# visinf/da-sac

Hardware: AMD Instinct MI355X
Metric: train images/sec (769x769, 19-cls, RN101 DeepLabv2, K=3) (higher is better)
Workload: dtype f32

## Files before the change

### da-sac_amd/csrc/conv_igemm.hip

```cpp
#include "common.hpp"

#include <atomic>
#include <cstdlib>
#include <type_traits>

namespace dasac {

typedef float f32x16 __attribute__((ext_vector_type(16)));
typedef float f32x4 __attribute__((ext_vector_type(4)));

constexpr int kBK = 16;
constexpr int kThreads = 256;
constexpr int kInvalid = 1 << 20;
constexpr int kSkWorkersPerCu = 3;
constexpr int kSkWorkers = kNumCu * kSkWorkersPerCu;
constexpr int kTileSlots = kNumCu * 4;
constexpr int kTailSlots = 2048;

#ifdef DASAC_TRACE_TILES
__device__ unsigned long long* g_tile_trace = nullptr;
__device__ __forceinline__ void trace_stamp(int slot) {
  if (g_tile_trace && threadIdx.x == 0) g_tile_trace[(size_t)blockIdx.x * 8 + slot] = __builtin_amdgcn_s_memtime();
}
#define DASAC_STAMP(slot) trace_stamp(slot)
#else
#define DASAC_STAMP(slot)
#endif

struct GemmGeom {
  int H, W, CxHW;
  int OH, OW, stride;
  int Npix;
  int n_tile0;
  int M, Mpad, Kpad;
  int OutH, OutW, ostride;
  unsigned x_bytes, w_bytes, z_bytes, out_bytes;
};

struct Epilogue {
  const float* shift;
  const float* res;
  const float* mask;
  int relu;
  const unsigned* mbits;
  unsigned* obits;
  int w32;
  float* stats;
};

constexpr unsigned kPoison = 0xFFFFFFFFu;
constexpr int64_t kMaxTensorBytes = (1ll << 32) - 4096;
constexpr int kRsrcFlags = 0x00020000;
typedef unsigned int u32x4 __attribute__((ext_vector_type(4)));

__device__ __forceinline__ __amdgpu_buffer_rsrc_t make_rsrc(const void* p, unsigned bytes) {
  return __builtin_amdgcn_make_buffer_rsrc(const_cast<void*>(p), 0, (int)bytes, kRsrcFlags);
}
__device__ __forceinline__ float buf_f32(__amdgpu_buffer_rsrc_t r, unsigned voff, int soff) {
  return __uint_as_float(__builtin_amdgcn_raw_buffer_load_b32(r, voff, soff, 0));
}

constexpr int kAuxSc1 = 16;
__device__ __forceinline__ f32x4 buf_f32x4_sc1(__amdgpu_buffer_rsrc_t r, unsigned voff, int soff) {
  const u32x4 v = __builtin_amdgcn_raw_buffer_load_b128(r, voff, soff, kAuxSc1);
  return f32x4{__uint_as_float(v.x), __uint_as_float(v.y), __uint_as_float(v.z), __uint_as_float(v.w)};
}
__device__ __forceinline__ f32x4 buf_f32x4(__amdgpu_buffer_rsrc_t r, unsigned voff, int soff) {
  const u32x4 v = __builtin_amdgcn_raw_buffer_load_b128(r, voff, soff, 0);
  return f32x4{__uint_as_float(v.x), __uint_as_float(v.y), __uint_as_float(v.z), __uint_as_float(v.w)};
}

#if __has_builtin(__builtin_amdgcn_writelane)
template <int LANE>
__device__ __forceinline__ int writelane_c(int val, int old) {
  return __builtin_amdgcn_writelane(val, LANE, old);
}
#else
extern "C" __device__ int dasac_llvm_writelane(int val, int lane, int old) __asm("llvm.amdgcn.writelane.i32");
template <int LANE>
__device__ __forceinline__ int writelane_c(int val, int old) {
  return dasac_llvm_writelane(val, LANE, old);
}
#endif
__device__ __forceinline__ int put_mask_rows(int rg, unsigned long long ballot, int acc) {
  const int lo = (int)(unsigned)ballot, hi = (int)(unsigned)(ballot >> 32);
  switch (rg) {
#define DASAC_ROW_(RG)                                               \
  case RG:                                                           \
    acc = writelane_c<(RG & 3) + 8 * (RG >> 2)>(lo, acc);            \
    acc = writelane_c<(RG & 3) + 8 * (RG >> 2) + 4>(hi, acc);        \
    break;
    DASAC_ROW_(0) DASAC_ROW_(1) DASAC_ROW_(2) DASAC_ROW_(3) DASAC_ROW_(4) DASAC_ROW_(5) DASAC_ROW_(6) DASAC_ROW_(7)
    DASAC_ROW_(8) DASAC_ROW_(9) DASAC_ROW_(10) DASAC_ROW_(11) DASAC_ROW_(12) DASAC_ROW_(13) DASAC_ROW_(14) DASAC_ROW_(15)
#undef DASAC_ROW_
  }
  return acc;
}

typedef __bf16 bf16x8 __attribute__((ext_vector_type(8)));
typedef __bf16 bf16x2 __attribute__((ext_vector_type(2)));
typedef float f32x2 __attribute__((ext_vector_type(2)));
__device__ __forceinline__ bf16x8 as_bf16x8(f32x4 v) { return __builtin_bit_cast(bf16x8, v); }
__device__ __forceinline__ unsigned pack_bf16(float a, float b) {
  return __builtin_bit_cast(unsigned, __builtin_convertvector((f32x2){a, b}, bf16x2));
}
__device__ __forceinline__ void split_bf16(f32x4 v0, f32x4 v1, f32x4& heads, f32x4& tails) {
  const float v[8] = {v0.x, v0.y, v0.z, v0.w, v1.x, v1.y, v1.z, v1.w};
#pragma unroll
  for (int p = 0; p < 4; ++p) {
    const unsigned h = pack_bf16(v[2 * p], v[2 * p + 1]);
    const float t0 = v[2 * p] - __uint_as_float(h << 16), t1 = v[2 * p + 1] - __uint_as_float(h & 0xffff0000u);
    heads[p] = __uint_as_float(h);
    tails[p] = __uint_as_float(pack_bf16(t0, t1));
  }
}

template <int CTRL>
__device__ __forceinline__ float dpp_add(float v) {
  return v + __int_as_float(__builtin_amdgcn_update_dpp(0, __float_as_int(v), CTRL, 0xf, 0xf, true));
}
__device__ __forceinline__ float half_wave_sum(float v) {
  v = dpp_add<0xB1>(v);
  v = dpp_add<0x4E>(v);
  v = dpp_add<0x141>(v);
  v = dpp_add<0x140>(v);
  return v + __shfl_xor(v, 16, 64);
}

template <int BM, int BN, int WAVES_M, int BK, bool FAST, int SK, bool X3, int BITS = 0>
__global__ __launch_bounds__(kThreads, SK == 1 ? kSkWorkersPerCu : 4) void conv_gemm(const float* __restrict__ X, const float* __restrict__ Wp,
                                                      const int4* __restrict__ tab, float* __restrict__ Out,
                                                      GemmGeom g, Epilogue ep, int m_tiles, int n_tiles,
                                                      float* __restrict__ partial, int* __restrict__ flags, int tail_tiles,
                                                      int tail_split) {
  constexpr bool STREAMK = SK == 1;
  constexpr bool TAIL = SK == 2;
  constexpr bool HANDOFF = STREAMK || TAIL;
  constexpr int WAVES_N = 4 / WAVES_M;
  constexpr int WM = BM / WAVES_M, WN = BN / WAVES_N;
  constexpr int TM = WM / 32, TN = WN / 32;
  constexpr int KQ = BK / 4;
  constexpr int A_VEC = KQ * BM;
  constexpr int A_PER_T = (A_VEC + kThreads - 1) / kThreads;
  constexpr int B_Q_PASS = kThreads / BN > 0 ? kThreads / BN : 1;
  constexpr int B_QUADS = KQ / B_Q_PASS;
  constexpr int ACC_REGS = TM * TN * 16;
  static_assert(TM >= 1 && TN >= 1 && BN <= kThreads && KQ % B_Q_PASS == 0, "tile shape");
  static_assert(!X3 || (BK == 16 && BN == 128), "split-bf16 path: one 16-deep MFMA block per K-step, a k octet per thread");

  __shared__ f32x4 sA[2][KQ * BM];
  __shared__ f32x4 sB[2][KQ * BN];
  __shared__ __attribute__((aligned(16))) float s_shift[BM];
  __shared__ unsigned s_vo[BN];
  __shared__ __attribute__((aligned(16))) unsigned s_mbits[BITS == 2 ? (BN / 32) * BM : 4];

  const int t = threadIdx.x, lane = t & 63;
  const int wave = __builtin_amdgcn_readfirstlane(t >> 6);
  const int wm = wave / WAVES_N, wn = wave % WAVES_N;
  const int li = lane & 31, lh = lane >> 5;

  const __amdgpu_buffer_rsrc_t rx = make_rsrc(X, g.x_bytes);
  const __amdgpu_buffer_rsrc_t rw = make_rsrc(Wp, g.w_bytes);

  const int OHW = g.OH * g.OW;
  const int planeHW = g.H * g.W;
  const int bcol = t % BN;
  const int bq0 = __builtin_amdgcn_readfirstlane(t / BN);
  const int a_step_bytes = KQ * g.Mpad * 16;
  const int KT = g.Kpad / BK;
  const int OutHW = g.OutH * g.OutW;
  const __amdgpu_buffer_rsrc_t ro = make_rsrc(Out, g.out_bytes);
  const __amdgpu_buffer_rsrc_t rres = make_rsrc(ep.res ? ep.res : Out, g.out_bytes);
  const __amdgpu_buffer_rsrc_t rmsk = BITS == 2 ? make_rsrc(ep.mbits, g.M * ep.w32 * 4) : make_rsrc(ep.mask ? ep.mask : Out, g.out_bytes);
  const __amdgpu_buffer_rsrc_t rsh = make_rsrc(ep.shift ? ep.shift : Out, ep.shift ? g.M * 4 : 0);
  const bool ragged = (g.M & 7) != 0;
  const __amdgpu_buffer_rsrc_t rpart = make_rsrc(HANDOFF ? (const void*)partial : (const void*)Out,
                                                 HANDOFF ? (STREAMK ? kSkWorkers : kTailSlots) * ACC_REGS * kThreads * 4 : 0);

  const int bid = blockIdx.x;
  const int xcd = bid % kNumXcd, slot = bid / kNumXcd;
  int it, it_end;
  int my_range = 0;
  int sk_per = 0, sk_rem = 0;
  auto sk_start = [&](int r) { return r * sk_per + min(r, sk_rem); };
  if (STREAMK) {
    const int G = gridDim.x;
    my_range = xcd * (G / kNumXcd) + slot;
    const int sk_total = m_tiles * n_tiles * KT;
    sk_per = sk_total / G;
    sk_rem = sk_total - sk_per * G;
    it = sk_start(my_range);
    it_end = sk_start(my_range + 1);
  } else {
    const int per_xcd = (n_tiles + kNumXcd - 1) / kNumXcd;
    const int lead_blocks = per_xcd * kNumXcd * m_tiles;
    if (!TAIL || bid < lead_blocks) {
      const int n_local = slot / m_tiles;
      const int n_tile = xcd * per_xcd + n_local;
      if (n_local >= per_xcd || n_tile >= n_tiles) return;
      it = (n_tile * m_tiles + slot % m_tiles) * KT;
      it_end = it + KT;
    } else {
      const int q = bid - lead_blocks;
      const int per_x = (tail_tiles + kNumXcd - 1) / kNumXcd;
      const int part_rev = q / (per_x * kNumXcd), ql = q - part_rev * (per_x * kNumXcd);
      const int tl = ql / kNumXcd;
      const int tr = xcd * per_x + tl;
      if (tr >= tail_tiles) return;
      const int part = tail_split - 1 - part_rev;
      const int tile = n_tiles * m_tiles + tr;
      it = tile * KT + part * KT / tail_split;
      it_end = tile * KT + (part + 1) * KT / tail_split;
      my_range = tr * (tail_split - 1) + part - 1;
    }
  }

  do {
    const int tile = it / KT;
    const int ks = it - tile * KT;
    const int ke = min(KT, ks + (it_end - it));
    it += ke - ks;
    const int m0 = (tile % m_tiles) * BM, n0 = (g.n_tile0 + tile / m_tiles) * BN;

    int pixbase, ih0, iw0;
    unsigned pro_vo = kPoison;
    {
      const int pix = n0 + bcol;
      if (pix < g.Npix) {
        const int n = pix / OHW, r = pix - n * OHW;
        const int oh = r / g.OW, ow = r - oh * g.OW;
        ih0 = oh * g.stride;
// ... 1197 lines not shown
  DASAC_REQUIRE(!stats || (!x3 && !mask_bits && !relu_bits_out && dasac_conv_gemm_bits_ok(M, Cx) && ostride == 1),
                "conv_gemm_stats: needs the 128-row fp32 tile with Cx %% 16 == 0 (dasac_conv_gemm_stats_ok), no bit masks");
  DASAC_REQUIRE(!(mask && mask_bits), "conv_gemm: give the ReLU pattern as fp32 mask OR as bit mask");
  DASAC_REQUIRE(!(mask_bits || relu_bits_out) || (ostride == 1 && OutH == OH && OutW == OW),
                "conv_gemm: bit masks index the GEMM's own pixel axis (ostride must be 1)");
  DASAC_REQUIRE(!relu_bits_out || relu, "conv_gemm: relu_bits_out records the pattern of a ReLU epilogue");
  DASAC_REQUIRE(!(x3 && (mask_bits || relu_bits_out)), "conv_gemm_x3: bit masks are implemented for the fp32 kernel only");
  DASAC_REQUIRE(!stats || (!res && !relu), "conv_gemm_stats: the statistics epilogue stores the raw convolution (+ shift): no residual, no ReLU");
  GemmGeom g;
  const int Mpad = dasac_conv_mpad(M), Kloop = (K + kBK - 1) / kBK * kBK;
  int rc = fill_geom(g, Nb, Cx, H, W, OH, OW, stride, M, Mpad, Kloop, OutH, OutW, ostride);
  if (rc) return rc;
  DASAC_REQUIRE((int64_t)dasac_conv_kpad(K) * Mpad * 4 < (1ll << 31), "conv: packed weights exceed 2 GiB");
  g.w_bytes = dasac_conv_kpad(K) * Mpad * 4;
  Epilogue ep{shift, res, mask, relu, mask_bits, relu_bits_out, (g.Npix + 31) / 32, stats};
  DASAC_REQUIRE((int64_t)M * ep.w32 * 4 < (1ll << 31), "conv_gemm: bit mask exceeds the 2 GiB buffer-descriptor window");
  const int4* tab = reinterpret_cast<const int4*>(table);
  hipStream_t s = as_stream(stream);
  const bool fast = Cx % kBK == 0;
  const int bm = pick_bm(Mpad);
  const int bn = bm == 32 ? 256 : 128;
  const int pix_end = pix_count > 0 ? pix_begin + pix_count : g.Npix;
  DASAC_REQUIRE(schedule >= 0 && schedule <= 2, "conv_gemm: schedule must be 0 (auto), 1 (tile per block) or 2 (stream-K)");
  DASAC_REQUIRE(pix_begin >= 0 && pix_begin < g.Npix && pix_begin % bn == 0 && pix_end > pix_begin && pix_end <= g.Npix &&
                    (pix_end == g.Npix || pix_end % bn == 0),
                "conv_gemm: pixel range [%d, %d) must consist of whole %d-pixel tiles", pix_begin, pix_end, bn);
  g.n_tile0 = pix_begin / bn;
  const int n_tiles = (pix_end - pix_begin + bn - 1) / bn;
  if (x3) {
    DASAC_REQUIRE(bm >= 64, "conv_gemm_x3: needs M > 32 (use dasac_conv_gemm for skinny outputs)");
    if (bm == 128)
      rc = fast ? launch_gemm<128, 128, 2, kBK, true, true>(x, packed, tab, out, g, ep, n_tiles, schedule, workspace, ws_bytes, s)
                : launch_gemm<128, 128, 2, kBK, false, true>(x, packed, tab, out, g, ep, n_tiles, schedule, workspace, ws_bytes, s);
    else
      rc = fast ? launch_gemm<64, 128, 2, kBK, true, true>(x, packed, tab, out, g, ep, n_tiles, 1, nullptr, 0, s)
                : launch_gemm<64, 128, 2, kBK, false, true>(x, packed, tab, out, g, ep, n_tiles, 1, nullptr, 0, s);
    if (rc) return rc;
    DASAC_CHECK_LAUNCH("conv_gemm_x3");
    return DASAC_OK;
  }
  if (stats) {
    rc = launch_gemm<128, 128, 2, kBK, true, false, 3>(x, packed, tab, out, g, ep, n_tiles, schedule, workspace, ws_bytes, s);
    if (rc) return rc;
    DASAC_CHECK_LAUNCH("conv_gemm_stats");
    return DASAC_OK;
  }
  if (mask_bits || relu_bits_out) {
    DASAC_REQUIRE(dasac_conv_gemm_bits_ok(M, Cx) && !(mask_bits && relu_bits_out),
                  "conv_gemm: bit masks need the 128-row fp32 tile with Cx %% 16 == 0 (dasac_conv_gemm_bits_ok), one direction per call");
    rc = relu_bits_out ? launch_gemm<128, 128, 2, kBK, true, false, 1>(x, packed, tab, out, g, ep, n_tiles, schedule, workspace, ws_bytes, s)
                       : launch_gemm<128, 128, 2, kBK, true, false, 2>(x, packed, tab, out, g, ep, n_tiles, schedule, workspace, ws_bytes, s);
    if (rc) return rc;
    DASAC_CHECK_LAUNCH("conv_gemm");
    return DASAC_OK;
  }
  switch (bm) {
    case 128:
      rc = fast ? launch_gemm<128, 128, 2, kBK, true>(x, packed, tab, out, g, ep, n_tiles, schedule, workspace, ws_bytes, s)
                : launch_gemm<128, 128, 2, kBK, false>(x, packed, tab, out, g, ep, n_tiles, schedule, workspace, ws_bytes, s);
      break;
    case 64:
      rc = fast ? launch_gemm<64, 128, 2, kBK, true>(x, packed, tab, out, g, ep, n_tiles, 1, nullptr, 0, s)
                : launch_gemm<64, 128, 2, kBK, false>(x, packed, tab, out, g, ep, n_tiles, 1, nullptr, 0, s);
      break;
    default:
      rc = fast ? launch_gemm<32, 256, 1, kBK, true>(x, packed, tab, out, g, ep, n_tiles, 1, nullptr, 0, s)
                : launch_gemm<32, 256, 1, kBK, false>(x, packed, tab, out, g, ep, n_tiles, 1, nullptr, 0, s);
      break;
  }
  if (rc) return rc;
  DASAC_CHECK_LAUNCH("conv_gemm");
  return DASAC_OK;
}

extern "C" int dasac_conv_gemm(const float* x, const float* packed, const int32_t* table, float* out, int Nb, int Cx,
                               int H, int W, int OH, int OW, int stride, int M, int K, int OutH, int OutW, int ostride,
                               const float* shift, const float* res, const float* mask, const uint32_t* mask_bits,
                               uint32_t* relu_bits_out, int relu, int pix_begin, int pix_count, int schedule,
                               void* workspace, size_t ws_bytes, dasac_stream_t stream) {
  return conv_gemm_impl(false, x, packed, table, out, Nb, Cx, H, W, OH, OW, stride, M, K, OutH, OutW, ostride, shift, res, mask,
                        mask_bits, relu_bits_out, relu, pix_begin, pix_count, schedule, workspace, ws_bytes, stream);
}

extern "C" int dasac_conv_gemm_stats_ok(int M, int Cx) { return dasac_conv_gemm_bits_ok(M, Cx); }
extern "C" int dasac_conv_gemm_stats_tiles(int Nb, int OH, int OW) { return (int)(((int64_t)Nb * OH * OW + 127) / 128); }
extern "C" int dasac_conv_gemm_stats(const float* x, const float* packed, const int32_t* table, float* out, int Nb, int Cx,
                                     int H, int W, int OH, int OW, int stride, int M, int K, int OutH, int OutW, int ostride,
                                     const float* shift, const float* res, int relu, int pix_begin, int pix_count, int schedule,
                                     void* workspace, size_t ws_bytes, float* stats, dasac_stream_t stream) {
  DASAC_REQUIRE(stats, "conv_gemm_stats: null statistics buffer");
  return conv_gemm_impl(false, x, packed, table, out, Nb, Cx, H, W, OH, OW, stride, M, K, OutH, OutW, ostride, shift, res, nullptr,
                        nullptr, nullptr, relu, pix_begin, pix_count, schedule, workspace, ws_bytes, stream, stats);
}

extern "C" int dasac_conv_gemm_x3(const float* x, const void* packed_x3, const int32_t* table, float* out, int Nb, int Cx,
                                  int H, int W, int OH, int OW, int stride, int M, int K, int OutH, int OutW, int ostride,
                                  const float* shift, const float* res, const float* mask, const uint32_t* mask_bits,
                                  uint32_t* relu_bits_out, int relu, int pix_begin, int pix_count, int schedule,
                                  void* workspace, size_t ws_bytes, dasac_stream_t stream) {
  return conv_gemm_impl(true, x, reinterpret_cast<const float*>(packed_x3), table, out, Nb, Cx, H, W, OH, OW, stride, M, K, OutH,
                        OutW, ostride, shift, res, mask, mask_bits, relu_bits_out, relu, pix_begin, pix_count, schedule, workspace,
                        ws_bytes, stream);
}

extern "C" int dasac_conv_pack_x3(const float* packed, int M, int K, void* packed_x3, dasac_stream_t stream) {
  DASAC_REQUIRE(packed && packed_x3, "conv_pack_x3: null pointer");
  const int Mpad = dasac_conv_mpad(M), Kpad = dasac_conv_kpad(K);
  hipLaunchKernelGGL(pack_x3, dim3(stream_grid((int64_t)(Kpad / 8) * Mpad, 256)), dim3(256), 0, as_stream(stream),
                     reinterpret_cast<const f32x4*>(packed), reinterpret_cast<f32x4*>(packed_x3), Mpad, Kpad);
  DASAC_CHECK_LAUNCH("pack_x3");
  return DASAC_OK;
}

static int wgrad_bn(int Cx) { return (Cx % 128 != 0 && Cx % 64 == 0) ? 64 : 128; }

static int wgrad_splits(int Mpad, int Kpad, int Npix, int BM, int BNk = 128) {
  const int tiles = (Mpad / BM) * (Kpad / BNk);
  const int slots = kNumCu * 3;
  constexpr int kMinPix = 256;
  int max_splits = (Npix + kMinPix - 1) / kMinPix;
  const int cap = (tiles < 12 && Npix >= 200000) ? (slots + tiles - 1) / tiles : 64;
  if (max_splits > cap) max_splits = cap;
  if (max_splits < 1) max_splits = 1;
  int best = 1;
  double best_eff = 0.0;
  for (int sp = 1; sp <= max_splits; ++sp) {
    const int blocks = tiles * sp;
    const int rounds = (blocks + slots - 1) / slots;
    const double eff = (double)blocks / ((double)rounds * slots);
    if (eff > best_eff + 0.02) {
      best_eff = eff;
      best = sp;
    }
  }
  return best;
}

extern "C" size_t dasac_conv_wgrad_workspace(int Nb, int OH, int OW, int M, int K) {
  const int Mpad = dasac_conv_mpad(M), Kpad = dasac_conv_kpad(K);
  const int s128 = wgrad_splits(Mpad, Kpad, Nb * OH * OW, pick_bm(Mpad), 128), s64 = wgrad_splits(Mpad, Kpad, Nb * OH * OW, pick_bm(Mpad), 64);
  const int splits = s128 > s64 ? s128 : s64;
  return (size_t)splits * Mpad * (Kpad + 1) * sizeof(float);
}

static int conv_wgrad_impl(bool x3, const float* dz, const float* x, const int32_t* table, int Nb, int Cx, int H, int W, int OH,
                           int OW, int stride, int M, int K, void* workspace, size_t ws_bytes, dasac_stream_t stream) {
  DASAC_REQUIRE(dz && x && table && workspace, "conv_wgrad: null pointer");
  GemmGeom g;
  const int Mpad = dasac_conv_mpad(M), Kpad = dasac_conv_kpad(K);
  int rc = fill_geom(g, Nb, Cx, H, W, OH, OW, stride, M, Mpad, Kpad, OH, OW, 1);
  if (rc) return rc;
  const int bm = pick_bm(Mpad);
  const int bnk = (M % 8 == 0 && bm != 32) ? wgrad_bn(Cx) : 128;
  const int splits = wgrad_splits(Mpad, Kpad, g.Npix, bm, bnk);
  if (ws_bytes < (size_t)splits * Mpad * (Kpad + 1) * sizeof(float)) return fail(DASAC_EWORKSPACE, "conv_wgrad: workspace too small");
  int per = (g.Npix + splits - 1) / splits;
  per = (per + kWgPix - 1) / kWgPix * kWgPix;
  const int4* tab = reinterpret_cast<const int4*>(table);
  float* P = reinterpret_cast<float*>(workspace);
  float* Psum = P + (size_t)splits * Mpad * Kpad;
  hipStream_t s = as_stream(stream);
  const bool fast = (Cx % 128 == 0) && (M % 8 == 0);
  if (bnk == 64) {
    if (bm == 128) launch_wgrad<128, 64, 2, true>(x3, dz, x, tab, P, Psum, g, splits, per, s);
    else launch_wgrad<64, 64, 2, true>(x3, dz, x, tab, P, Psum, g, splits, per, s);
    DASAC_CHECK_LAUNCH("conv_wgrad");
// ... 208 lines not shown
```

### da-sac_amd/dasac_hip/lib.py

```python
import ctypes as C
import os

import torch

LIB_PATH = os.environ.get("DASAC_LIB") or os.path.join(os.path.dirname(os.path.abspath(__file__)), "libdasac_hip.so")

_p, _i, _l, _f, _sz = C.c_void_p, C.c_int, C.c_int64, C.c_float, C.c_size_t

PROTOTYPES = {
    "dasac_version": (_i, []),
    "dasac_last_error": (C.c_char_p, []),
    "dasac_device_info": (_i, [C.POINTER(_i), C.POINTER(_i), C.c_char_p, _sz]),
    "dasac_reserved_cus": (_i, []),
    "dasac_set_reserved_cus": (_i, [_i]),
    "dasac_pseudo_labels_workspace": (_sz, [_i, _i, _l]),
    "dasac_pseudo_labels": (_i, [_p, _p, _p, _f, _f, _i, _i, _l, _p, _p, _p, _p, _sz, _p]),
    "dasac_conv_mpad": (_i, [_i]),
    "dasac_conv_kpad": (_i, [_i]),
    "dasac_conv_table": (_i, [_p, _p, _p, _p, _i, _i, _i, _i, _i, _i, _p, _p]),
    "dasac_conv_pack": (_i, [_p, _p, _i, _i, _i, _i, _i, _i, _i, _p, _p]),
    "dasac_relu_bits_words": (_sz, [_i, _l]),
    "dasac_conv_gemm_bits_ok": (_i, [_i, _i]),
    "dasac_conv_gemm": (_i, [_p, _p, _p, _p] + [_i] * 12 + [_p, _p, _p, _p, _p, _i, _i, _i, _i, _p, _sz, _p]),
    "dasac_conv_gemm_x3": (_i, [_p, _p, _p, _p] + [_i] * 12 + [_p, _p, _p, _p, _p, _i, _i, _i, _i, _p, _sz, _p]),
    "dasac_conv_pack_x3": (_i, [_p, _i, _i, _p, _p]),
    "dasac_conv_gemm_workspace": (_sz, []),
    "dasac_conv_gemm_schedule": (_i, [_i, _i, _i, _i, _i]),
    "dasac_conv_gemm_tail_split": (_i, [_i, _i, _i, _i, _i]),
    "dasac_conv_wgrad_workspace": (_sz, [_i, _i, _i, _i, _i]),
    "dasac_conv_wgrad": (_i, [_p, _p, _p] + [_i] * 9 + [_p, _sz, _p]),
    "dasac_conv_wgrad_x3": (_i, [_p, _p, _p] + [_i] * 9 + [_p, _sz, _p]),
    "dasac_upsample_softmax": (_i, [_p, _i, _i, _i, _i, _i, _i, _p, _p, _p, _p, _p]),
    "dasac_infer_labels": (_i, [_p, _i, _i, _i, _i, _i, _i, _p, _p, _p, _p]),
    "dasac_image_pyramid": (_i, [_p, _i, _i, _i, _i, _i, _i, _i, _p, _p]),
    "dasac_infer_fuse": (_i, [_p, _i, _i, _i, _i, _i, _i, _p, _p, _p, _p, _p]),
    "dasac_upsample_bwd_workspace": (_sz, [_i, _i, _i]),
    "dasac_upsample_bwd": (_i, [_p, _i, _i, _i, _i, _i, _p, _p, _p, _sz, _p]),
    "dasac_ce_loss_workspace": (_sz, [_i, _i, _l]),
    "dasac_ce_loss": (_i, [_p, _p, _p, _p, _i, _i, _l, _i, _p, _p, _p, _p, _p, _sz, _p]),
    "dasac_ce_loss_bwd_low_workspace": (_sz, [_i, _i, _i, _i]),
    "dasac_ce_loss_bwd_low": (_i, [_p, _p, _p, _p, _i, _i, _i, _i, _i, _i, _i, _p, _p, _p, _sz, _p]),
    "dasac_warp_affine": (_i, [_p, _p, _i, _i, _i, _i, _p, _p]),
    "dasac_warp_pool": (_i, [_p, _p, _p, _i, _i, _i, _i, _i, _i, _f, _p, _p, _p, _p]),
    "dasac_warp_back": (_i, [_p, _p, _p, _i, _i, _i, _i, _i, _p, _p]),
    "dasac_class_state": (_i, [_p, _p, _i, _l, _i, _f, _f, _i, _f, _p, _p, _p]),
    "dasac_bn_fold": (_i, [_p, _p, _p, _p, _p, _f, _i, _p, _p, _p, _p]),
    "dasac_bn_param_grads": (_i, [_p, _i, _p, _p, _p, _p, _p, _i, _p, _p, _p, _p]),
    "dasac_channel_sums": (_i, [_p, _i, _i, _l, _p, _p]),
    "dasac_maxpool_fwd": (_i, [_p, _i, _i, _i, _i, _i, _i, _i, _i, _p, _p, _p]),
    "dasac_maxpool_bwd": (_i, [_p, _p, _p, _i, _i, _i, _i, _i, _i, _i, _i, _i, _p, _p]),
    "dasac_ema_chunk_elems": (_i, []),
    "dasac_ema_update": (_i, [_p, _i, _p, _i, _f, _i, _p, _p, _p]),
    "dasac_sgd_step": (_i, [_p, _i, _p, _i, _p, _p, _i, _f, _i, _p]),
    "dasac_sgd_nesterov_step": (_i, [_p, _i, _p, _i, _p, _p, _i, _f, _i, _p]),
    "dasac_adam_step": (_i, [_p, _i, _p, _i, _p, _i, C.c_double, C.c_double, C.c_double, _p]),
    "dasac_grad_norm_workspace": (_sz, [_i]),
    "dasac_grad_norm": (_i, [_p, _i, _i, _p, _i, _f, _p, _sz, _p, _p, _p]),
    "dasac_sgd_step_ctl": (_i, [_p, _i, _p, _i, _p, _p, _i, _f, _i, _p, _i, _i, _p]),
    "dasac_sgd_nesterov_step_ctl": (_i, [_p, _i, _p, _i, _p, _p, _i, _f, _i, _p, _i, _i, _p]),
    "dasac_adam_step_ctl": (_i, [_p, _i, _p, _i, _p, _i, C.c_double, C.c_double, C.c_double, _p, _i, _i, _p]),
    "dasac_scale_planes": (_i, [_p, _p, _l, _l, _p, _p]),
    "dasac_add": (_i, [_p, _p, _p, _l, _p]),
    "dasac_relu_mask": (_i, [_p, _p, _p, _l, _p]),
    "dasac_bn_stats_workspace": (_sz, [_i, _i, _l]),
    "dasac_bn_stats": (_i, [_p, _i, _i, _l, _p, _p, _sz, _p]),
    "dasac_bn_train_finalize": (_i, [_p, C.c_double, _p, _p, _p, _p, _p, _p, _f, _f, _i, _p, _p, _p, _p, _p]),
    "dasac_bn_apply": (_i, [_p, _p, _p, _p, _i, _i, _i, _l, _p, _p]),
    "dasac_bn_bwd_reduce": (_i, [_p, _p, _p, _p, _i, _i, _l, _p, _p, _p, _p, _sz, _p]),
    "dasac_bn_train_finalize_tiles": (_i, [_p, _i, _i, C.c_double, _p, _p, _p, _p, _p, _f, _f, _i, _p, _p, _p, _p, _p]),
    "dasac_bn_tile_stats_reduce": (_i, [_p, _i, _i, _i, _p, _p]),
    "dasac_bn_train_apply_tiles": (_i, [_p, _p, _i, _i, C.c_double, _p, _p, _p, _p, _p, _f, _f, _p, _i, _i, _i, _l, _p, _p, _p, _p]),
    "dasac_bn_bwd_fused": (_i, [_p, _p, _p, _p, _p, C.c_double, _i, _i, _l, _p, _p, _p, _p, _sz, _p]),
    "dasac_conv_gemm_stats_ok": (_i, [_i, _i]),
    "dasac_conv_gemm_stats_tiles": (_i, [_i, _i, _i]),
    "dasac_conv_gemm_stats": (_i, [_p, _p, _p, _p] + [_i] * 12 + [_p, _p, _i, _i, _i, _i, _p, _sz, _p, _p]),
    "dasac_bn_bwd_apply": (_i, [_p, _p, _p, _p, _p, _p, C.c_double, _p, _i, _i, _l, _p, _p, _p, _p]),
    "dasac_winograd_tiles": (_i, [_i, _i, _i, _i]),
    "dasac_winograd_filter": (_i, [_p, _p, _i, _i, _i, _p, _p]),
    "dasac_winograd_input": (_i, [_p, _i, _i, _i, _i, _i, _p, _sz, _p]),
    "dasac_winograd_output": (_i, [_p, _sz, _i, _i, _i, _i, _i, _p, _i, _p, _p, _p, _p]),
    "dasac_conv_pack_expanded":(_i, [_p, _i, _i, _i, _i, _i, _i, _i, _p, _p]),
    "dasac_tap_gather": (_i, [_p, _p, _p, _p, _p, _i, _i, _i, _p, _i, _i, _i, _p, _p]),
    "dasac_tap_scatter": (_i, [_p, _p, _p, _p, _p, _i, _i, _i, _i, _i, _i, _p, _p]),
    "dasac_conv_wgrad_finish_expanded": (_i, [_p, _i, _i, _i, _i, _i, _p, _i, _i, _i, _i, _p]),
    "dasac_pack_chunk_elems": (_i, []),
    "dasac_bn_fold_multi": (_i, [_p, _p, _i, _p]),
    "dasac_conv_pack_multi": (_i, [_p, _p, _i, _p]),
    "dasac_label_pad_mask": (_i, [_p, _p, _l, _i, _i, _p]),
    "dasac_dropout_planes": (_i, [C.c_uint64, C.c_uint64, _f, _l, _p, _p]),
    "dasac_iou_counts": (_i, [_p, _p, _i, _i, _l, _i, _p, _p]),
    "dasac_mask_counts": (_i, [_p, _p, _p, _p, _p, _p, _p, _i, _i, _l, _i, _p, _p]),
    "dasac_label_hist": (_i, [_p, _i, _l, _p, _p]),
    "dasac_make_views_table_ints": (_i, [_i, _i]),
    "dasac_make_views": (_i, [_p, _p, _p, _i, _i, _i, _p, _p, _p, _i, _p, _p, _p, _p]),
    "dasac_view_photometric_workspace": (_sz, [_i, _i, _i]),
    "dasac_view_photometric": (_i, [_p, _p, _i, _i, _i, _p, _p, _p, _i, _p, _p, _p, _sz, _p]),
    "dasac_conv_wgrad_dot_rows": (_i, [_i, _i]),
    "dasac_conv_wgrad_finish": (_i, [_p, _i, _i, _i, _i, _i, _p, _p, _p, _p, _p, _i, _i, _i, _p]),
    "dasac_crop_table_ints": (_i, [_i, _i]),
    "dasac_resize_u8": (_i, [_p, _l, _p, _l, _i, _p, _p, _l, _i, _p, _l, _p, _l, _p]),
    "dasac_make_crops": (_i, [_p, _l, _p, _l, _i, _p, _p, _l, _i, _i, _p, _p, _i, _p, _p, _p, _p, _p, _p]),
    "dasac_vis_panels": (_i, [_p, _p, _i, _i, _i, _i, _i, _p, _p, _p, _p, _p, _p, _p]),
    "dasac_vis_grid": (_i, [_p, _i, _i, _i, _i, _f, _p, _p]),
}


# ... 102 lines not shown
```

### da-sac_amd/dasac_hip/ops.py

```python
import os

import torch

from . import lib as L


def _c(t):
    return t if t.is_contiguous() else t.contiguous()


class _Profile:

    def __init__(self):
        self.on, self.records = False, []

    def start(self):
        self.on, self.records = True, []

    def stop(self, by_shape=False):
        self.on = False
        torch.cuda.synchronize()
        out = {}
        for name, flops, a, b, tag, nbytes in self.records:
            d = out.setdefault((name, tag) if by_shape else name, {"flops": 0.0, "bytes": 0.0, "seconds": 0.0, "launches": 0})
# ... 113 lines not shown
        tap0 += kh * kw


def conv_pack(spec, weights, transposed, scale=None, out=None, order=0):
    lib = L.load()
    L.require_gpu(*weights)
    M = spec.cin if transposed else spec.cout
    K = spec.Kt if transposed else spec.K
    shape = (lib.dasac_conv_kpad(K), lib.dasac_conv_mpad(M))
    if out is None:
        out = torch.empty(shape, dtype=torch.float32, device=weights[0].device)
    for w, (taps, tap0) in zip(weights, _branch_taps(spec)):
        L.check(lib.dasac_conv_pack(_c(w).data_ptr(), L.ptr(scale), spec.cout, spec.cin, taps, tap0, spec.taps,
                                    int(transposed), int(order), out.data_ptr(), L.stream_ptr()), "dasac_conv_pack")
    return _finish_pack(out, M, K)


def bits_ok(M, Cx):
    return PRECISION == "fp32" and bool(L.load().dasac_conv_gemm_bits_ok(int(M), int(Cx)))


class ReluBits:

    def __init__(self, Nb, M, OH, OW, device):
        self.shape = (Nb, M, OH, OW)
        self.words = torch.empty(L.load().dasac_relu_bits_words(M, Nb * OH * OW), dtype=torch.int32, device=device)


def stats_ok(M, Cx):
    return PRECISION == "fp32" and bool(L.load().dasac_conv_gemm_stats_ok(int(M), int(Cx)))


def tile_stats_buffer(Nb, M, OH, OW, device):
    lib = L.load()
    return torch.empty((lib.dasac_conv_gemm_stats_tiles(Nb, OH, OW), 2, lib.dasac_conv_mpad(M)), dtype=torch.float32, device=device)


def conv_gemm(x, packed, table, out, grid_hw, stride, M, K, ostride=1, shift=None, res=None, mask=None, relu=False, bits_out=None,
              stats=None, schedule=None):
    lib = L.load()
    L.require_gpu(x, packed, table, out)
    Nb, Cx, H, W = x.shape
    OH, OW = grid_hw
    assert out.shape[0] == Nb and out.shape[1] == M and x.is_contiguous() and out.is_contiguous()
    mask_bits = None
    if isinstance(mask, ReluBits):
        assert mask.shape == tuple(out.shape) and ostride == 1
        mask_bits, mask = mask.words, None
    if bits_out is not None:
        assert relu and ostride == 1 and bits_out.shape == tuple(out.shape)
    for t_ in (res, mask):
        assert t_ is None or (t_.shape == out.shape and t_.is_contiguous())
    ws = L.workspace(lib.dasac_conv_gemm_workspace(), x.device, owner="conv_gemm")
    fn = lib.dasac_conv_gemm_x3 if getattr(packed, "dasac_x3", False) else lib.dasac_conv_gemm
    tag = (M, K, Nb * OH * OW, stride, ostride, res is not None, mask is not None or mask_bits is not None)

    n = Nb * OH * OW
    nbytes = 4.0 * (x.numel() + packed.numel() + n * M * (1 + (res is not None) + (mask is not None)
                                                          + ((mask_bits is not None) + (bits_out is not None)) / 32.0))

    def launch(span, schedule):
        with PROFILE.span(span, 2.0 * n * M * K, tag, nbytes):
            if stats is not None:
                assert mask is None and mask_bits is None and bits_out is None and stats.is_contiguous() and stats.dtype == torch.float32
                L.check(lib.dasac_conv_gemm_stats(x.data_ptr(), packed.data_ptr(), table.data_ptr(), out.data_ptr(), Nb, Cx, H, W, OH, OW,
                                                  stride, M, K, out.shape[2], out.shape[3], ostride, L.ptr(shift), L.ptr(res), int(relu),
                                                  0, 0, schedule, L.ptr(ws), 0 if ws is None else ws.numel(),
                                                  stats.data_ptr(), L.stream_ptr()), "dasac_conv_gemm_stats")
            else:
                L.check(fn(x.data_ptr(), packed.data_ptr(), table.data_ptr(), out.data_ptr(), Nb, Cx, H, W, OH, OW,
                           stride, M, K, out.shape[2], out.shape[3], ostride, L.ptr(shift), L.ptr(res),
                           L.ptr(mask), L.ptr(mask_bits), 0 if bits_out is None else bits_out.words.data_ptr(), int(relu),
                           0, 0, schedule, L.ptr(ws), 0 if ws is None else ws.numel(),
                           L.stream_ptr()), "dasac_conv_gemm")

    if schedule is not None:
        launch("conv_gemm<stream-K>" if schedule == 2 else "conv_gemm<tile-per-block>", int(schedule))
        return out
    if lib.dasac_conv_gemm_tail_split(Nb, OH, OW, M, K) > 0:
        launch("conv_gemm<tile+tail>", 0)
        return out
    sk = PROFILE.on and lib.dasac_conv_gemm_schedule(Nb, OH, OW, M, K)
    launch("conv_gemm<stream-K>" if sk else "conv_gemm<tile-per-block>", 0)
    return out


def conv_forward(spec, x, weights, scale=None, shift=None, res=None, relu=False, table=None, packed=None):
    Nb, _, H, W = x.shape
    OH, OW = spec.out_hw(H, W)
    order = gemm_order(spec, False)
    table = conv_table(spec, H, W, False, x.device, order) if table is None else table
    packed = conv_pack(spec, weights, False, scale, order=order) if packed is None else packed
    out = torch.empty((Nb, spec.cout, OH, OW), dtype=torch.float32, device=x.device)
    return conv_gemm(x, packed, table, out, (OH, OW), spec.stride, spec.cout, spec.K, 1, shift, res, None, relu)


def conv_dgrad(spec, dz, weights, in_hw, scale=None, res=None, mask=None, table=None, packed=None):
    Nb, _, OH, OW = dz.shape
    H, W = in_hw
    order = gemm_order(spec, True)
    table = conv_table(spec, OH, OW, True, dz.device, order) if table is None else table
    packed = conv_pack(spec, weights, True, scale, order=order) if packed is None else packed
    if spec.stride == 1:
        dx = torch.empty((Nb, spec.cin, H, W), dtype=torch.float32, device=dz.device)
        return conv_gemm(dz, packed, table, dx, (H, W), 1, spec.cin, spec.Kt, 1, None, res, mask, False)
    assert spec.taps == 1 and spec.branches[0][3] == 0, "strided data-gradient only for 1x1 convolutions"
    if res is None:
        dx = torch.empty((Nb, spec.cin, H, W), dtype=torch.float32, device=dz.device)
        dx.zero_()
    else:
        dx = res
    assert not isinstance(mask, ReluBits), "strided data gradient: the pattern is applied by relu_mask on the fp32 activation"
    conv_gemm(dz, packed, table, dx, (OH, OW), 1, spec.cin, spec.Kt, spec.stride, None,
              dx if res is not None else None, None, False)
    return relu_mask(dx, mask) if mask is not None else dx


ALGORITHM = "auto"
WINOGRAD_MIN_CHANNEL_PRODUCT = 512 * 512
_MAX_TENSOR_BYTES = (1 << 32) - 4096


def set_conv_algorithm(mode):
    global ALGORITHM
    assert mode in ("auto", "direct"), mode
    ALGORITHM = mode


def winograd_ok(spec, transposed=False):
    if len(spec.branches) != 1 or spec.stride != 1 or PRECISION != "fp32":
        return False
    kh, kw, d, p = spec.branches[0]
    C = spec.cout if transposed else spec.cin
    return kh == 3 and kw == 3 and d >= 1 and p == d and C % 16 == 0


def winograd_routed(spec, transposed, Nb, H, W):
    if ALGORITHM != "auto" or not winograd_ok(spec, transposed) or spec.cin * spec.cout < WINOGRAD_MIN_CHANNEL_PRODUCT:
        return False
    T = L.load().dasac_winograd_tiles(Nb, H, W, spec.branches[0][2])
    return T > 0 and 64 * max(spec.cin, spec.cout) * T <= _MAX_TENSOR_BYTES


def winograd_filter(spec, weight, transposed, scale=None, out=None):
    lib = L.load()
    L.require_gpu(weight, scale)
    M, K = (spec.cin, spec.cout) if transposed else (spec.cout, spec.cin)
    shape = (16, lib.dasac_conv_kpad(K), lib.dasac_conv_mpad(M))
    if out is None or tuple(out.shape) != shape:
        out = torch.empty(shape, dtype=torch.float32, device=weight.device)
    L.check(lib.dasac_winograd_filter(_c(weight).data_ptr(), L.ptr(scale), spec.cout, spec.cin, int(transposed), out.data_ptr(),
                                      L.stream_ptr()), "dasac_winograd_filter")
    return out


_wino_tables = {}


def _winograd_table(C, T, device):
    key = (device.index, C, T)
    t = _wino_tables.get(key)
    if t is None:
        if len(_wino_tables) > 64:
            _wino_tables.clear()
        t = _wino_tables[key] = conv_table(ConvSpec(C, C, [(1, 1, 1, 0)]), 1, T, False, device)
    return t


def winograd_output(y, out, dilation, shift=None, relu=False, mask_bits=None, bits_out=None):
    lib = L.load()
    L.require_gpu(y, out, shift)
    Nb, M, H, W = out.shape
    assert y.is_contiguous() and out.is_contiguous() and y.dtype == torch.float32
    for b in (mask_bits, bits_out):
        assert b is None or b.shape == tuple(out.shape)
    with PROFILE.span("winograd_output", 0.0, None, 4.0 * (y.numel() + out.numel())):
        L.check(lib.dasac_winograd_output(y.data_ptr(), y.numel() * 4, Nb, M, H, W, int(dilation), L.ptr(shift), int(relu),
                                          0 if mask_bits is None else mask_bits.words.data_ptr(),
                                          0 if bits_out is None else bits_out.words.data_ptr(), out.data_ptr(), L.stream_ptr()),
                "dasac_winograd_output")
    return out


def winograd_conv(x, u, out, dilation, shift=None, relu=False, mask_bits=None, bits_out=None, gemm_schedule="auto"):
    lib = L.load()
    L.require_gpu(x, u, out)
    Nb, C, H, W = x.shape
    M = out.shape[1]
    assert x.is_contiguous() and out.is_contiguous() and tuple(out.shape) == (Nb, M, H, W)
    assert tuple(u.shape) == (16, lib.dasac_conv_kpad(C), lib.dasac_conv_mpad(M)) and u.is_contiguous()
    T = lib.dasac_winograd_tiles(Nb, H, W, int(dilation))
    if T <= 0 or 64 * max(C, M) * T > _MAX_TENSOR_BYTES:
        raise L.DasacError("winograd_conv: [16, {}, tiles] exceeds the 4 GiB buffer-descriptor window".format(max(C, M)))
    v_elems, y_elems = 16 * C * T, 16 * M * T
    ws = L.workspace(4 * (v_elems + y_elems), x.device)[:4 * (v_elems + y_elems)].view(torch.float32)
    v, y = ws[:v_elems].view(16, C, T), ws[v_elems:v_elems + y_elems].view(16, M, T)
    with PROFILE.span("winograd_input", 0.0, None, 4.0 * (x.numel() + v_elems)):
        L.check(lib.dasac_winograd_input(x.data_ptr(), Nb, C, H, W, int(dilation), v.data_ptr(), v_elems * 4, L.stream_ptr()),
                "dasac_winograd_input")
    table = _winograd_table(C, T, x.device)
    if gemm_schedule == "auto":
        gemm_schedule = 2 if ((M + 127) // 128) * ((T + 127) // 128) < 4 * L.EXPECTED_CUS else None
    for pt in range(16):
        conv_gemm(v[pt].view(1, C, 1, T), u[pt], table, y[pt].view(1, M, 1, T), (1, T), 1, M, C, schedule=gemm_schedule)
    return winograd_output(y, out, dilation, shift, relu, mask_bits, bits_out)


def dot_rows(spec):
    return L.load().dasac_conv_wgrad_dot_rows(spec.cin, spec.taps)


def conv_wgrad(spec, dz, x, weights, scale=None, dot=None, table=None, sum_dz=None, outs=None):
    lib = L.load()
    L.require_gpu(dz, x, *weights)
    assert dot is None or (tuple(dot.shape) == (dot_rows(spec), spec.cout) and dot.is_contiguous())
    Nb, Cx, H, W = x.shape
    _, M, OH, OW = dz.shape
    table = conv_table(spec, H, W, False, x.device) if table is None else table
    nbytes = lib.dasac_conv_wgrad_workspace(Nb, OH, OW, M, spec.K)
    ws = L.workspace(nbytes, x.device)
    with PROFILE.span("conv_wgrad", 2.0 * Nb * OH * OW * M * spec.K, (M, spec.K, Nb * OH * OW, spec.stride, 1, False, False),
                      4.0 * (dz.numel() + x.numel() + M * spec.K)):
        fn = lib.dasac_conv_wgrad_x3 if PRECISION == "bf16x3" else lib.dasac_conv_wgrad
        L.check(fn(_c(dz).data_ptr(), x.data_ptr(), table.data_ptr(), Nb, Cx, H, W, OH, OW, spec.stride, M,
                   spec.K, ws.data_ptr(), ws.numel(), L.stream_ptr()), "dasac_conv_wgrad")
    grads = [_dest(None if outs is None else outs[bi], w) for bi, w in enumerate(weights)]
    for w, dw, (taps, tap0) in zip(weights, grads, _branch_taps(spec)):
        L.check(lib.dasac_conv_wgrad_finish(ws.data_ptr(), Nb, OH, OW, M, spec.K, _c(w).data_ptr(), L.ptr(scale),
                                            dw.data_ptr(), L.ptr(dot), L.ptr(sum_dz if tap0 == 0 else None), spec.cin, taps,
                                            tap0, L.stream_ptr()),
                "dasac_conv_wgrad_finish")
    return grads


def _f32(shape, like):
    return torch.empty(shape, dtype=torch.float32, device=like.device)


def _dest(out, like):
    if out is None:
        return torch.empty_like(like, memory_format=torch.contiguous_format)
    assert out.dtype == torch.float32 and out.is_contiguous() and out.numel() == like.numel() and out.device == like.device
    return out


def upsample_softmax(logits, size, ignore=None, want_up=True, want_probs=False, want_sums=False):
    lib = L.load()
    L.require_gpu(logits, ignore)
    logits = _c(logits)
    B, Cn, h, w = logits.shape
    H, W = int(size[0]), int(size[1])
    up = _f32((B, Cn, H, W), logits) if want_up else None
    probs = _f32((B, Cn, H, W), logits) if want_probs else None
    sums = torch.empty(Cn, dtype=torch.float64, device=logits.device) if want_sums else None
    ign = None if ignore is None else _c(ignore).view(torch.uint8)
    with PROFILE.span("upsample_softmax", 0.0, None, logits.numel() * 4.0 + B * Cn * H * W * 4.0 * (int(want_up) + int(want_probs)) + (B * H * W if ignore is not None else 0)):
        L.check(lib.dasac_upsample_softmax(logits.data_ptr(), B, Cn, h, w, H, W, L.ptr(ign), L.ptr(up), L.ptr(probs),
                                           L.ptr(sums), L.stream_ptr()), "dasac_upsample_softmax")
    return up, probs, sums


def infer_labels(logits, size, lut=None, want_conf=False):
    lib = L.load()
    L.require_gpu(logits, lut)
    logits = _c(logits)
    B, Cn, h, w = logits.shape
    H, W = int(size[0]), int(size[1])
    labels = torch.empty((B, H, W), dtype=torch.uint8, device=logits.device)
    conf = _f32((B, H, W), logits) if want_conf else None
    if lut is not None:
        assert lut.dtype == torch.uint8 and lut.numel() >= Cn and lut.is_contiguous()
    L.check(lib.dasac_infer_labels(logits.data_ptr(), B, Cn, h, w, H, W, L.ptr(lut), labels.data_ptr(), L.ptr(conf),
                                   L.stream_ptr()), "dasac_infer_labels")
    return labels, conf


INFER_MAX_SOURCES = 8
INFER_MODES = {"mean": 0, "max": 1}


def image_pyramid(image, size, flip=False):
    lib = L.load()
    L.require_gpu(image)
    if image.dtype != torch.float32 or image.dim() != 4:
        raise L.DasacError("image_pyramid takes a float32 [B,Cin,H,W] image (got {} {})".format(image.dtype, tuple(image.shape)))
    image = _c(image)
    B, Cin, H, W = image.shape
# ... 676 lines not shown
```

### include/dasac_hip.h

```cpp
#ifndef DASAC_HIP_H
#define DASAC_HIP_H

#include <stddef.h>
#include <stdint.h>

#ifdef __cplusplus
extern "C" {
#endif

#define DASAC_OK 0
#define DASAC_EINVAL (-1)
#define DASAC_EWORKSPACE (-2)
#define DASAC_ELAUNCH (-3)

typedef void* dasac_stream_t;

int dasac_version(void);
const char* dasac_last_error(void);
int dasac_device_info(int* cu_count, int* wave_size, char* arch, size_t arch_len);
int dasac_reserved_cus(void);
int dasac_set_reserved_cus(int n);

size_t dasac_pseudo_labels_workspace(int B, int C, int64_t HW);
int dasac_pseudo_labels(const float* probs, const uint8_t* ignore, const float* disc,
                        float upper, float lower, int B, int C, int64_t HW,
                        int64_t* labels, float* max_conf, int64_t* max_idx,
                        void* workspace, size_t ws_bytes, dasac_stream_t stream);

int dasac_conv_mpad(int M);
int dasac_conv_kpad(int K);
int dasac_conv_table(const int32_t* kh, const int32_t* kw, const int32_t* dil, const int32_t* pad,
                     int n_branches, int C, int plane_h, int plane_w, int transposed, int order,
                     int32_t* table, dasac_stream_t stream);
int dasac_conv_pack(const float* w, const float* scale, int Cout, int Cin, int taps, int tap0,
                    int total_taps, int transposed, int order, float* packed, dasac_stream_t stream);
size_t dasac_relu_bits_words(int M, int64_t Npix);
int dasac_conv_gemm_bits_ok(int M, int Cx);
int dasac_conv_gemm(const float* x, const float* packed, const int32_t* table, float* out,
                    int Nb, int Cx, int H, int W, int OH, int OW, int stride, int M, int K,
                    int OutH, int OutW, int ostride,
                    const float* shift, const float* res, const float* mask,
                    const uint32_t* mask_bits, uint32_t* relu_bits_out,
                    int relu, int pix_begin, int pix_count, int schedule,
                    void* workspace, size_t ws_bytes, dasac_stream_t stream);
int dasac_conv_pack_x3(const float* packed, int M, int K, void* packed_x3, dasac_stream_t stream);
int dasac_conv_gemm_x3(const float* x, const void* packed_x3, const int32_t* table, float* out,
                       int Nb, int Cx, int H, int W, int OH, int OW, int stride, int M, int K,
                       int OutH, int OutW, int ostride,
                       const float* shift, const float* res, const float* mask,
                       const uint32_t* mask_bits, uint32_t* relu_bits_out,
                       int relu, int pix_begin, int pix_count, int schedule,
                       void* workspace, size_t ws_bytes, dasac_stream_t stream);
int dasac_conv_gemm_stats_ok(int M, int Cx);
int dasac_conv_gemm_stats_tiles(int Nb, int OH, int OW);
int dasac_conv_gemm_stats(const float* x, const float* packed, const int32_t* table, float* out,
                          int Nb, int Cx, int H, int W, int OH, int OW, int stride, int M, int K,
                          int OutH, int OutW, int ostride, const float* shift, const float* res, int relu,
                          int pix_begin, int pix_count, int schedule, void* workspace, size_t ws_bytes,
                          float* stats, dasac_stream_t stream);
size_t dasac_conv_gemm_workspace(void);
int dasac_conv_gemm_schedule(int Nb, int OH, int OW, int M, int K);
int dasac_conv_gemm_tail_split(int Nb, int OH, int OW, int M, int K);
size_t dasac_conv_wgrad_workspace(int Nb, int OH, int OW, int M, int K);
int dasac_conv_wgrad(const float* dz, const float* x, const int32_t* table,
                     int Nb, int Cx, int H, int W, int OH, int OW, int stride, int M, int K,
                     void* workspace, size_t ws_bytes, dasac_stream_t stream);
int dasac_conv_wgrad_x3(const float* dz, const float* x, const int32_t* table,
                        int Nb, int Cx, int H, int W, int OH, int OW, int stride, int M, int K,
                        void* workspace, size_t ws_bytes, dasac_stream_t stream);
int dasac_conv_wgrad_dot_rows(int Cin, int taps);
int dasac_conv_wgrad_finish(const void* workspace, int Nb, int OH, int OW, int M, int K,
                            const float* w, const float* scale, float* dw, float* dot,
                            float* sum_dz, int Cin, int taps, int tap0, dasac_stream_t stream);

int dasac_winograd_tiles(int Nb, int H, int W, int dilation);
int dasac_winograd_filter(const float* w, const float* scale, int Cout, int Cin, int transposed, float* u,
                          dasac_stream_t stream);
int dasac_winograd_input(const float* x, int Nb, int C, int H, int W, int dilation, float* v, size_t v_bytes,
                         dasac_stream_t stream);
int dasac_winograd_output(const float* y, size_t y_bytes, int Nb, int M, int H, int W, int dilation, const float* shift,
                          int relu, const uint32_t* mask_bits, uint32_t* relu_bits_out, float* out, dasac_stream_t stream);

int dasac_conv_pack_expanded(const float* w, int Cout, int Cin, int taps, int tap0, int total_taps,
                             int Cp, int transposed, float* packed, dasac_stream_t stream);
int dasac_tap_gather(const float* y, const int32_t* kh, const int32_t* kw, const int32_t* dil,
                     const int32_t* pad, int n_branches, int Cp, int Cout, const float* bias, int B,
                     int H, int W, float* out, dasac_stream_t stream);
int dasac_tap_scatter(const float* dout, const int32_t* kh, const int32_t* kw, const int32_t* dil,
                      const int32_t* pad, int n_branches, int Cp, int Cout, int B, int H, int W,
                      float* d, dasac_stream_t stream);
int dasac_conv_wgrad_finish_expanded(const void* workspace, int Nb, int OH, int OW, int E, int Cin,
                                     float* dw, int Cout, int taps, int tap0, int Cp,
                                     dasac_stream_t stream);

int dasac_upsample_softmax(const float* logits, int B, int C, int h, int w, int H, int W,
                           const uint8_t* ignore, float* up, float* probs, double* class_sums,
                           dasac_stream_t stream);
size_t dasac_upsample_bwd_workspace(int planes, int H, int w);
int dasac_upsample_bwd(const float* grad_up, int planes, int h, int w, int H, int W,
                       const float* gscale, float* grad_low, void* workspace, size_t ws_bytes,
                       dasac_stream_t stream);
size_t dasac_ce_loss_workspace(int B, int C, int64_t HW);
int dasac_ce_loss(const float* logits, const int64_t* labels, const float* class_weight,
                  const float* conf, int B, int C, int64_t HW, int mode, const float* gscale,
                  float* loss, float* dlogits, float* per_class, void* workspace, size_t ws_bytes,
                  dasac_stream_t stream);
size_t dasac_ce_loss_bwd_low_workspace(int B, int C, int H, int w);
int dasac_ce_loss_bwd_low(const float* logits_up, const int64_t* labels, const float* class_weight, const float* conf,
                          int B, int C, int H, int W, int h, int w, int mode, const float* gscale, float* grad_low,
                          void* workspace, size_t ws_bytes, dasac_stream_t stream);
int dasac_infer_labels(const float* logits, int B, int C, int h, int w, int H, int W, const uint8_t* lut,
                       uint8_t* labels, float* conf, dasac_stream_t stream);
#define DASAC_INFER_MAX_SOURCES 8
#define DASAC_INFER_MEAN 0
#define DASAC_INFER_MAX 1
typedef struct dasac_infer_source {
  const float* logits;
  int32_t h, w, flip, reserved;
} dasac_infer_source;
int dasac_image_pyramid(const float* image, int B, int Cin, int H, int W, int Hs, int Ws, int with_flip, float* out,
                        dasac_stream_t stream);
int dasac_infer_fuse(const dasac_infer_source* sources, int n_sources, int B, int C, int H, int W, int mode,
                     const uint8_t* lut, uint8_t* labels, float* conf, float* probs, dasac_stream_t stream);
int dasac_warp_affine(const float* x, const float* theta, int B, int C, int H, int W, float* out,
                      dasac_stream_t stream);
int dasac_warp_pool(const float* probs, const float* theta, const float* theta_inv, int N, int T,
                    int C, int H, int W, int mode, float tolerance, float* aligned, float* pooled,
// ... 151 lines not shown
```

Before: 20.63.

## Batch the sixteen Winograd point GEMMs into one grid-y launch

Adds a batched variant of the tile-per-block fp32 conv GEMM kernel, where blockIdx.y selects one of the per-point Winograd GEMMs through per-batch strides on input, weights and output. The Winograd path now issues one launch for all sixteen transform points when the schedule is auto and padded M fits the 128-row tile, instead of sixteen sequential launches that used a stream-K or tail schedule for small grids. The aim is to cut launch overhead and fill the GPU with more blocks at once. In exchange, the small-problem stream-K/tail scheduling is dropped for these GEMMs, and the batched path has no epilogue options.

```diff
diff --git a/da-sac_amd/csrc/conv_igemm.hip b/da-sac_amd/csrc/conv_igemm.hip
--- a/da-sac_amd/csrc/conv_igemm.hip
+++ b/da-sac_amd/csrc/conv_igemm.hip
@@ -46,6 +46,10 @@
   unsigned* obits;
   int w32;
   float* stats;
+};
+
+struct BatchedEpilogue : Epilogue {
+  int64_t x_stride, w_stride, out_stride;
 };
 
 constexpr unsigned kPoison = 0xFFFFFFFFu;
@@ -130,7 +134,8 @@
 template <int BM, int BN, int WAVES_M, int BK, bool FAST, int SK, bool X3, int BITS = 0>
 __global__ __launch_bounds__(kThreads, SK == 1 ? kSkWorkersPerCu : 4) void conv_gemm(const float* __restrict__ X, const float* __restrict__ Wp,
                                                       const int4* __restrict__ tab, float* __restrict__ Out,
-                                                      GemmGeom g, Epilogue ep, int m_tiles, int n_tiles,
+                                                      GemmGeom g, std::conditional_t<BITS == 4, BatchedEpilogue, Epilogue> ep,
+                                                      int m_tiles, int n_tiles,
                                                       float* __restrict__ partial, int* __restrict__ flags, int tail_tiles,
                                                       int tail_split) {
   constexpr bool STREAMK = SK == 1;
@@ -147,6 +152,13 @@
   constexpr int ACC_REGS = TM * TN * 16;
   static_assert(TM >= 1 && TN >= 1 && BN <= kThreads && KQ % B_Q_PASS == 0, "tile shape");
   static_assert(!X3 || (BK == 16 && BN == 128), "split-bf16 path: one 16-deep MFMA block per K-step, a k octet per thread");
+  static_assert(BITS != 4 || (SK == 0 && FAST && !X3 && BM == 128), "batched launch: the plain fp32 tile-per-block kernel only");
+  if constexpr (BITS == 4) {
+    const int64_t b = blockIdx.y;
+    X += b * ep.x_stride;
+    Wp += b * ep.w_stride;
+    Out += b * ep.out_stride;
+  }
 
   __shared__ f32x4 sA[2][KQ * BM];
   __shared__ f32x4 sB[2][KQ * BN];
@@ -1510,6 +1522,40 @@
                         mask_bits, relu_bits_out, relu, pix_begin, pix_count, schedule, workspace, ws_bytes, stream);
 }
 
+extern "C" int dasac_conv_gemm_batched(const float* x, const float* packed, const int32_t* table, float* out, int Nb, int Cx,
+                                       int H, int W, int OH, int OW, int stride, int M, int K, int OutH, int OutW, int ostride,
+                                       int batch, int64_t x_stride, int64_t packed_stride, int64_t out_stride,
+                                       dasac_stream_t stream) {
+  DASAC_REQUIRE(batch >= 1 && batch <= 65535, "conv_gemm_batched: batch %d outside 1..65535 (grid y)", batch);
+  DASAC_REQUIRE(x && packed && table && out, "conv_gemm_batched: null pointer");
+  DASAC_REQUIRE(Cx > 0 && Cx % kBK == 0, "conv_gemm_batched: gathered channels %d must be a multiple of %d", Cx, kBK);
+  GemmGeom g;
+  const int Mpad = dasac_conv_mpad(M), Kloop = (K + kBK - 1) / kBK * kBK;
+  DASAC_REQUIRE(pick_bm(Mpad) == 128, "conv_gemm_batched: needs the 128-row tile (padded M = %d)", Mpad);
+  int rc = fill_geom(g, Nb, Cx, H, W, OH, OW, stride, M, Mpad, Kloop, OutH, OutW, ostride);
+  if (rc) return rc;
+  const int64_t w_elems = (int64_t)dasac_conv_kpad(K) * Mpad;
+  DASAC_REQUIRE(w_elems * 4 < (1ll << 31), "conv: packed weights exceed 2 GiB");
+  g.w_bytes = (unsigned)(w_elems * 4);
+  const int64_t x_elems = (int64_t)Nb * Cx * H * W, out_elems = (int64_t)Nb * M * OutH * OutW;
+  if (batch > 1 || x_stride || packed_stride || out_stride) {
+    DASAC_REQUIRE(x_stride >= x_elems && packed_stride >= w_elems && out_stride >= out_elems,
+                  "conv_gemm_batched: a per-batch stride is smaller than one entry (x %lld < %lld, packed %lld < %lld or out %lld < %lld)",
+                  (long long)x_stride, (long long)x_elems, (long long)packed_stride, (long long)w_elems, (long long)out_stride,
+                  (long long)out_elems);
+    DASAC_REQUIRE(x_stride % 4 == 0 && packed_stride % 4 == 0 && out_stride % 4 == 0,
+                  "conv_gemm_batched: per-batch strides must be multiples of 4 elements (16-byte aligned entries)");
+  }
+  const int n_tiles = (g.Npix + 127) / 128, m_tiles = (M + 127) / 128;
+  if ((long long)m_tiles * (n_tiles + kNumXcd) * (g.Kpad / kBK) >= (1ll << 31)) return fail(DASAC_EINVAL, "conv_gemm: iteration space exceeds 2^31");
+  BatchedEpilogue ep{{nullptr, nullptr, nullptr, 0, nullptr, nullptr, (g.Npix + 31) / 32, nullptr}, x_stride, packed_stride, out_stride};
+  const int n_tiles_pad = (n_tiles + kNumXcd - 1) / kNumXcd * kNumXcd;
+  hipLaunchKernelGGL((conv_gemm<128, 128, 2, kBK, true, 0, false, 4>), dim3(n_tiles_pad * m_tiles, batch), dim3(kThreads), 0,
+                     as_stream(stream), x, packed, reinterpret_cast<const int4*>(table), out, g, ep, m_tiles, n_tiles, nullptr, nullptr, 0, 1);
+  DASAC_CHECK_LAUNCH("conv_gemm_batched");
+  return DASAC_OK;
+}
+
 extern "C" int dasac_conv_gemm_stats_ok(int M, int Cx) { return dasac_conv_gemm_bits_ok(M, Cx); }
 extern "C" int dasac_conv_gemm_stats_tiles(int Nb, int OH, int OW) { return (int)(((int64_t)Nb * OH * OW + 127) / 128); }
 extern "C" int dasac_conv_gemm_stats(const float* x, const float* packed, const int32_t* table, float* out, int Nb, int Cx,
diff --git a/da-sac_amd/dasac_hip/lib.py b/da-sac_amd/dasac_hip/lib.py
--- a/da-sac_amd/dasac_hip/lib.py
+++ b/da-sac_amd/dasac_hip/lib.py
@@ -22,6 +22,7 @@
     "dasac_relu_bits_words": (_sz, [_i, _l]),
     "dasac_conv_gemm_bits_ok": (_i, [_i, _i]),
     "dasac_conv_gemm": (_i, [_p, _p, _p, _p] + [_i] * 12 + [_p, _p, _p, _p, _p, _i, _i, _i, _i, _p, _sz, _p]),
+    "dasac_conv_gemm_batched": (_i, [_p, _p, _p, _p] + [_i] * 12 + [_i, _l, _l, _l, _p]),
     "dasac_conv_gemm_x3": (_i, [_p, _p, _p, _p] + [_i] * 12 + [_p, _p, _p, _p, _p, _i, _i, _i, _i, _p, _sz, _p]),
     "dasac_conv_pack_x3": (_i, [_p, _i, _i, _p, _p]),
     "dasac_conv_gemm_workspace": (_sz, []),
diff --git a/da-sac_amd/dasac_hip/ops.py b/da-sac_amd/dasac_hip/ops.py
--- a/da-sac_amd/dasac_hip/ops.py
+++ b/da-sac_amd/dasac_hip/ops.py
@@ -219,6 +219,25 @@
         return out
     sk = PROFILE.on and lib.dasac_conv_gemm_schedule(Nb, OH, OW, M, K)
     launch("conv_gemm<stream-K>" if sk else "conv_gemm<tile-per-block>", 0)
+    return out
+
+
+def conv_gemm_batched(x, packed, table, out, grid_hw, stride, M, K, ostride=1, strides=None):
+    lib = L.load()
+    L.require_gpu(x, packed, table, out)
+    B, Nb, Cx, H, W = x.shape
+    OH, OW = grid_hw
+    assert out.shape[:3] == (B, Nb, M) and packed.shape[0] == B and packed.dtype == x.dtype == out.dtype == torch.float32
+    for t_ in (x, packed, out):
+        assert t_[:1].is_contiguous()
+    sx, sw, so = (x.stride(0), packed.stride(0), out.stride(0)) if strides is None else strides
+    n = Nb * OH * OW
+    tag = (M, K, n, stride, ostride, B)
+    nbytes = 4.0 * (x.numel() + packed.numel() + B * n * M)
+    with PROFILE.span("conv_gemm<batched>", 2.0 * B * n * M * K, tag, nbytes):
+        L.check(lib.dasac_conv_gemm_batched(x.data_ptr(), packed.data_ptr(), table.data_ptr(), out.data_ptr(), Nb, Cx, H, W, OH, OW,
+                                            stride, M, K, out.shape[3], out.shape[4], ostride, B, sx, sw, so, L.stream_ptr()),
+                "dasac_conv_gemm_batched")
     return out
 
 
@@ -336,10 +355,13 @@
         L.check(lib.dasac_winograd_input(x.data_ptr(), Nb, C, H, W, int(dilation), v.data_ptr(), v_elems * 4, L.stream_ptr()),
                 "dasac_winograd_input")
     table = _winograd_table(C, T, x.device)
+    if gemm_schedule == "auto" and lib.dasac_conv_mpad(M) % 128 != 0:
+        gemm_schedule = None
     if gemm_schedule == "auto":
-        gemm_schedule = 2 if ((M + 127) // 128) * ((T + 127) // 128) < 4 * L.EXPECTED_CUS else None
-    for pt in range(16):
-        conv_gemm(v[pt].view(1, C, 1, T), u[pt], table, y[pt].view(1, M, 1, T), (1, T), 1, M, C, schedule=gemm_schedule)
+        conv_gemm_batched(v.view(16, 1, C, 1, T), u, table, y.view(16, 1, M, 1, T), (1, T), 1, M, C)
+    else:
+        for pt in range(16):
+            conv_gemm(v[pt].view(1, C, 1, T), u[pt], table, y[pt].view(1, M, 1, T), (1, T), 1, M, C, schedule=gemm_schedule)
     return winograd_output(y, out, dilation, shift, relu, mask_bits, bits_out)
 
 
diff --git a/include/dasac_hip.h b/include/dasac_hip.h
--- a/include/dasac_hip.h
+++ b/include/dasac_hip.h
@@ -43,6 +43,11 @@
                     const uint32_t* mask_bits, uint32_t* relu_bits_out,
                     int relu, int pix_begin, int pix_count, int schedule,
                     void* workspace, size_t ws_bytes, dasac_stream_t stream);
+int dasac_conv_gemm_batched(const float* x, const float* packed, const int32_t* table, float* out,
+                            int Nb, int Cx, int H, int W, int OH, int OW, int stride, int M, int K,
+                            int OutH, int OutW, int ostride,
+                            int batch, int64_t x_stride, int64_t packed_stride, int64_t out_stride,
+                            dasac_stream_t stream);
 int dasac_conv_pack_x3(const float* packed, int M, int K, void* packed_x3, dasac_stream_t stream);
 int dasac_conv_gemm_x3(const float* x, const void* packed_x3, const int32_t* table, float* out,
                        int Nb, int Cx, int H, int W, int OH, int OW, int stride, int M, int K,
```

After: 20.97 (median of 6 runs). 1.02x the previous value.
